# markdl/mtcp

Hardware: AMD Instinct MI355X
Metric: device-resident Gpkt/s + payload GB/s checksummed, 1/2/4/8 MI355X (higher is better)
Workload: dtype u8

## Files before the change

### mtcp_amd/csrc/dispatch.hpp

```cpp
#pragma once

#include <stdint.h>
#include <stdlib.h>
#include <string.h>

#include "../../include/mtcp_gpu.h"

namespace {

enum Sched : int { kSchedAuto = 0, kSchedWave, kSchedRow, kSchedQuad, kSchedBig, kSchedSpan, kSchedOct };

constexpr uint64_t kQuadOnlyUpToSlot = 64;
constexpr uint64_t kSpanUpToSlot = 640;
constexpr uint32_t kOctUpToPkts = 1u << 16;
constexpr uint64_t kOctUpToSlot = 2048;

inline int sched_from_env() {
    const char *e = getenv("MTCP_GPU_SCHED");
    if (!e) return kSchedAuto;
    if (!strcmp(e, "wave")) return kSchedWave;
    if (!strcmp(e, "row")) return kSchedRow;
    if (!strcmp(e, "quad")) return kSchedQuad;
    if (!strcmp(e, "span")) return kSchedSpan;
    if (!strcmp(e, "oct")) return kSchedOct;
    if (!strcmp(e, "big")) return kSchedBig;
    return kSchedAuto;
}

constexpr uint64_t kSpanNarrowUpToSlot = 896;
constexpr uint64_t kWaveNarrowUpToSlot = 4096;
constexpr uint32_t kWaveNarrowFromPkts = 1u << 20;

inline bool narrow_batch(const mtcp_gpu_size_hint *h) {
    if (!h || h->min_len == 0 || h->max_len < h->min_len) return false;
    const uint32_t lo = ((uint32_t)h->min_len + 63) & ~63u, hi = ((uint32_t)h->max_len + 63) & ~63u;
    return hi <= 2 * lo;
}

inline int pick_sched(int forced, uint32_t n, uint64_t slot, bool small_only, bool rx, bool narrow = false) {
    int s = forced;
    if (s == kSchedAuto) {
        int big = slot <= kQuadOnlyUpToSlot ? kSchedQuad
                  : slot <= kSpanUpToSlot   ? kSchedSpan
                  : (n <= kOctUpToPkts && slot <= kOctUpToSlot) ? kSchedOct : kSchedBig;
        if (narrow && slot > kQuadOnlyUpToSlot && slot <= kSpanUpToSlot && n <= kOctUpToPkts)
            big = kSchedOct;
        else if (narrow && slot > kSpanUpToSlot && slot <= kSpanNarrowUpToSlot && n > kOctUpToPkts)
            big = kSchedSpan;
        if (slot < 256) {
            s = n <= 2048 ? kSchedWave : n <= (1u << 17) ? kSchedQuad : big;
        } else if (narrow && slot <= kSpanUpToSlot && n > 2048 && n <= kOctUpToPkts) {
            s = kSchedOct;
        } else if (narrow && slot <= 320 && n > 2048 && n <= (1u << 17)) {
            s = kSchedQuad;
        } else if (slot >= 4096) {
            s = n <= (1u << 16) || (narrow && slot <= kWaveNarrowUpToSlot && n >= kWaveNarrowFromPkts)
                    ? kSchedWave : kSchedBig;
        } else {
            s = n <= 8192 || (slot >= 2048 && n <= 16384) ? kSchedWave
                : n <= (1u << 15)                          ? kSchedRow : big;
        }
    }
    if (s == kSchedSpan && !rx) s = kSchedBig;
    if (s == kSchedBig && small_only) s = kSchedRow;
    return s;
}

constexpr uint64_t kWaveShortUpToSlot = 2048;

constexpr uint64_t kUnrollBelowSlotBytes = 1024;
constexpr uint64_t kLineAlignAboveSlotBytes = 1536;
constexpr uint32_t kSortedUpToPkts = 1u << 16;

enum BigSched : int { kBigSorted = 0, kBigUnrolled, kBigUnrolledLineAligned, kBigSortedLineAligned };

inline int big_schedule(bool ptrs, uint64_t slot, uint32_t batch_n) {
    if (ptrs) return kBigSortedLineAligned;
    if (slot < kUnrollBelowSlotBytes || (batch_n <= kSortedUpToPkts && slot <= kLineAlignAboveSlotBytes))
        return kBigSorted;
    return slot > kLineAlignAboveSlotBytes ? kBigUnrolledLineAligned : kBigUnrolled;
}

inline const char *kernel_name(int sched, int big, uint64_t slot) {
    switch (sched) {
        case kSchedWave: return slot <= kWaveShortUpToSlot ? "rx_wave_kernel<2 loads>" : "rx_wave_kernel<10 loads>";
        case kSchedQuad: return "rx_group_kernel<quad>";
        case kSchedOct: return "rx_group_kernel<oct>";
        case kSchedSpan: return "rx_span_kernel";
        case kSchedRow: return "rx_group_kernel<row>";
        default: break;
    }
    switch (big) {
        case kBigSorted: return "rx_kernel<sorted>";
        case kBigUnrolled: return "rx_kernel<unrolled>";
        case kBigUnrolledLineAligned: return "rx_kernel<unrolled,line-aligned>";
        default: return "rx_kernel<sorted,line-aligned>";
    }
}

constexpr uint64_t kTxBuildOctUpToPayload = 48;
constexpr uint64_t kTxBuildRowUpToPayload = 384;
constexpr uint64_t kTxBuildHalfUpToPayload = 4096;
inline int txbuild_group(uint64_t payload_bytes, uint32_t n) {
    const uint64_t avg = n ? payload_bytes / n : 0;
    return avg <= kTxBuildOctUpToPayload    ? 8
           : avg <= kTxBuildRowUpToPayload  ? 16
           : avg <= kTxBuildHalfUpToPayload ? 32 : 64;
}

}
```

### mtcp_amd/csrc/mtcp_gpu.hip

```cpp
#include <hip/hip_runtime.h>
#include <stddef.h>
#include <stdint.h>
#include <string.h>

#include <algorithm>
#include <mutex>
#include <new>
#include <vector>

#include "../../include/mtcp_gpu.h"
#include "../../include/mtcp_gpu_flowtab.h"
#include "../../include/mtcp_gpu_group.h"
#include "../../include/mtcp_gpu_rcvwalk.h"
#include "../../include/mtcp_gpu_steer.h"
#include "../../include/mtcp_gpu_tcpopt.h"
#include "../../include/mtcp_gpu_txbuild.h"
#include "../../include/mtcp_gpu_txseg.h"
#include "ctx_internal.hpp"
#include "dispatch.hpp"
#include "flow_kernels.hpp"
#include "flowtab_kernels.hpp"
#include "group_kernels.hpp"
#include "host_call.hpp"
#include "host_copy.hpp"
#include "park.hpp"
#include "rcvwalk_kernels.hpp"
#include "rx_kernels.hpp"
#include "rx_span.hpp"
#include "steer_kernels.hpp"
#include "tcpopt_kernels.hpp"
#include "txbuild_kernels.hpp"
#include "txseg_kernels.hpp"
#include "wait.hpp"

namespace {

using namespace mtcp_host;
using mtcp_wait::Deadline;
using mtcp_wait::drain;

}

struct mtcp_gpu_ctx {
    int device = 0;
    int num_cu = 256;
    uint32_t flags = 0;
    uint32_t rss_nq = 1;
    uint32_t rss_endian = 0;
    uint32_t rss_key_w[4] = {0, 0, 0, 0};
    int sched = 0;
    hipStream_t stream = nullptr;
    const uint32_t *d_rss_tables = nullptr;
    uint32_t wait_us = 0;
    Stage stage[kStages];
    uint8_t *h_gather = nullptr;
    uint64_t h_gather_cap = 0;
    mtcp_gpu_desc *h_gather_desc = nullptr;
    uint32_t h_gather_desc_cap = 0;
    const char *last_kernel = "";
    bool abandoned = false;
};

namespace {

void build_rss_tables(const uint8_t key[40], uint32_t *tables) {
    uint32_t cache[96];
    uint32_t result = ((uint32_t)key[0] << 24) | ((uint32_t)key[1] << 16) |
                      ((uint32_t)key[2] << 8) | (uint32_t)key[3];
    uint32_t idx = 32;
    for (int i = 0; i < 96; i++, idx++) {
        cache[i] = result;
        const uint32_t bit = ((key[idx / 8] << (idx % 8)) & 0x80) ? 1u : 0u;
        result = (result << 1) | bit;
    }
    for (int t = 0; t < 24; ++t)
        for (int v = 0; v < 16; ++v) {
            uint32_t h = 0;
            for (int m = 0; m < 4; ++m)
                if (v & (0x8 >> m)) h ^= cache[4 * t + m];
            tables[t * 16 + v] = h;
        }
}

uint32_t grid_for(const mtcp_gpu_ctx *ctx, uint32_t n) {
    const uint32_t groups = (n + mg::kWave - 1) / mg::kWave;
    const uint32_t blocks = (groups + mg::kWavesPerBlock - 1) / mg::kWavesPerBlock;
    const uint32_t cap = (uint32_t)ctx->num_cu * 2;
    return std::max(1u, std::min(blocks, cap));
}

template <int SCHED, bool LALIGN>
constexpr int prio_for() { return SCHED == mg::kSchedUnrolled && !LALIGN ? 5 : 0; }

template <int MODE, bool RSS, int SCHED, bool LALIGN, bool CMP>
void launch_one(dim3 grid, dim3 block, hipStream_t st, const mg::KParams &kp) {
    constexpr bool kNT = MODE != mg::kTxChunk;
    constexpr bool kRev = LALIGN && SCHED == mg::kSchedUnrolled;
    constexpr int kB = SCHED == mg::kSchedSorted && !LALIGN && MODE == mg::kRxChunk ? 16 : 8;
    hipLaunchKernelGGL((mg::rx_kernel<MODE, RSS, SCHED, LALIGN, 0, 8, kB, kNT, 6, kRev, false,
                                      prio_for<SCHED, LALIGN>(), mg::kWavesPerBlock, 0, CMP>),
                       grid, block, 0, st, kp);
}

template <int MODE, bool RSS, bool CMP>
const char *launch_sched(dim3 grid, dim3 block, hipStream_t st, const mg::KParams &kp, uint64_t slot,
                         uint32_t batch_n) {
    const int b = big_schedule(MODE == mg::kRxPtrs, slot, batch_n);
    if constexpr (MODE == mg::kRxPtrs) {
        launch_one<MODE, RSS, mg::kSchedSorted, true, CMP>(grid, block, st, kp);
    } else if (b == kBigSorted) {
        launch_one<MODE, RSS, mg::kSchedSorted, false, CMP>(grid, block, st, kp);
    } else if (b == kBigUnrolledLineAligned) {
        launch_one<MODE, RSS, mg::kSchedUnrolled, true, CMP>(grid, block, st, kp);
    } else {
        launch_one<MODE, RSS, mg::kSchedUnrolled, false, CMP>(grid, block, st, kp);
    }
    return kernel_name(kSchedBig, b, slot);
}

constexpr uint32_t kHeldPasses = 8;


template <int MODE, bool RSS>
const char *launch_small(int sched, uint32_t n, uint64_t slot, hipStream_t st, const mg::KParams &kp) {
    if (sched == kSchedWave) {
        const dim3 grid((n + mg::kWavesPerBlock - 1) / mg::kWavesPerBlock);
        if (slot <= kWaveShortUpToSlot) {
            hipLaunchKernelGGL((mg::rx_wave_kernel<MODE, RSS, 0, 1, 2>), grid, dim3(mg::kBlock), 0, st, kp);
            return "rx_wave_kernel<2 loads>";
        }
        hipLaunchKernelGGL((mg::rx_wave_kernel<MODE, RSS>), grid, dim3(mg::kBlock), 0, st, kp);
        return "rx_wave_kernel<10 loads>";
    } else if (sched == kSchedQuad) {
        constexpr int kBlk = mg::kQuadBlock;
        constexpr uint32_t P = mg::GroupShape<4, kBlk>::P;
        hipLaunchKernelGGL((mg::rx_group_kernel<MODE, RSS, 4, 0, 1, kBlk>), dim3((n + P - 1) / P), dim3(kBlk), 0,
                           st, kp);
        return "rx_group_kernel<quad>";
    } else if (sched == kSchedOct) {
        constexpr int kBlk = mg::kOctBlock;
        constexpr uint32_t P = mg::GroupShape<8, kBlk>::P;
        hipLaunchKernelGGL((mg::rx_group_kernel<MODE, RSS, 8, 0, 1, kBlk>), dim3((n + P - 1) / P), dim3(kBlk), 0,
                           st, kp);
        return "rx_group_kernel<oct>";
    } else if (sched == kSchedSpan) {
        if constexpr (!mg::is_tx(MODE)) {
            hipLaunchKernelGGL((mg::rx_span_kernel<MODE, RSS>), dim3((n + mg::kSpanP - 1) / mg::kSpanP),
                               dim3(mg::kSpanBlock), 0, st, kp);
            return "rx_span_kernel";
        }
    }
    constexpr uint32_t P = mg::GroupShape<16>::P;
    hipLaunchKernelGGL((mg::rx_group_kernel<MODE, RSS, 16>), dim3((n + P - 1) / P), dim3(mg::kGroupBlock), 0,
                       st, kp);
    return "rx_group_kernel<row>";
}

uint64_t record_size(const mg::KParams &kp) { return kp.compact ? 16 : 40; }
uint64_t record_size(const mtcp_gpu_ctx *ctx) { return (ctx->flags & MTCP_GPU_F_COMPACT) ? 16 : 40; }

template <int MODE>
int launch(mtcp_gpu_ctx *ctx, const mg::KParams &kp, hipStream_t st, const mtcp_gpu_size_hint *hint = nullptr) {
    if (ctx->abandoned) return MTCP_GPU_EIO;
    if (kp.n == 0) return MTCP_GPU_OK;
    const bool rss = !mg::is_tx(MODE) && (ctx->flags & MTCP_GPU_F_RSS);
    const bool ptrs = MODE == mg::kRxPtrs || MODE == mg::kTxPtrs;
    const uint64_t avg_slot = ptrs ? 1024 : kp.buf_len / kp.n;
    const int sched = pick_sched(ctx->sched, kp.n, avg_slot, MODE == mg::kTxPtrs || kp.tx_report != nullptr,
                                 !mg::is_tx(MODE), !ptrs && narrow_batch(hint));
    if (sched != kSchedBig) {
        ctx->last_kernel = rss ? launch_small<MODE, true>(sched, kp.n, avg_slot, st, kp)
                               : launch_small<MODE, false>(sched, kp.n, avg_slot, st, kp);
        return HIP_OK(hipGetLastError()) ? MTCP_GPU_OK : MTCP_GPU_EIO;
    }
    if constexpr (MODE != mg::kTxPtrs) {
    const dim3 grid(grid_for(ctx, kp.n)), block(mg::kBlock);
    const uint64_t slot = kp.n ? kp.buf_len / kp.n : 0;
    const uint32_t cap = grid.x * mg::kWavesPerBlock * mg::kWave * kHeldPasses;
    for (uint32_t first = 0; first < kp.n; first += cap) {
        mg::KParams sub = kp;
        sub.n = std::min(kp.n - first, cap);
        if (MODE == mg::kRxPtrs) {
            sub.ptrs = kp.ptrs + first;
            sub.lens = kp.lens + first;
        } else {
            sub.desc = kp.desc + first;
        }
        if (MODE != mg::kTxChunk)
            sub.out = reinterpret_cast<mtcp_gpu_result *>(reinterpret_cast<uint8_t *>(kp.out) +
                                                          (uint64_t)first * record_size(kp));
        if (kp.bins) sub.bins = kp.bins + first;
        if constexpr (mg::is_tx(MODE)) {
            ctx->last_kernel = launch_sched<MODE, false, false>(grid, block, st, sub, slot, kp.n);
        } else if (kp.compact) {
            ctx->last_kernel = rss ? launch_sched<MODE, true, true>(grid, block, st, sub, slot, kp.n)
                                   : launch_sched<MODE, false, true>(grid, block, st, sub, slot, kp.n);
        } else {
            ctx->last_kernel = rss ? launch_sched<MODE, true, false>(grid, block, st, sub, slot, kp.n)
                                   : launch_sched<MODE, false, false>(grid, block, st, sub, slot, kp.n);
        }
    }
    }
    return HIP_OK(hipGetLastError()) ? MTCP_GPU_OK : MTCP_GPU_EIO;
}

mg::KParams base_params(mtcp_gpu_ctx *ctx) {
    mg::KParams kp{};
    kp.rss_tables = ctx->d_rss_tables;
    kp.rss_nq = ctx->rss_nq;
    kp.rss_endian = ctx->rss_endian;
    for (int i = 0; i < 4; ++i) kp.rss_key[i] = ctx->rss_key_w[i];
    kp.compact = (ctx->flags & MTCP_GPU_F_COMPACT) ? 1u : 0u;
    return kp;
}

uintptr_t out_align(const mtcp_gpu_ctx *ctx) { return (ctx->flags & MTCP_GPU_F_COMPACT) ? 15 : 7; }

hipStream_t pick(mtcp_gpu_ctx *ctx, void *stream) {
    return stream ? reinterpret_cast<hipStream_t>(stream) : ctx->stream;
}

void stage_release_buf(Stage &s, bool may_free) {
    mtcp_park::release(s.d_buf, s.buf_cap, mtcp_park::kDevice, may_free);
    s.d_buf = nullptr;
    s.buf_cap = 0;
}
void stage_release_pkts(Stage &s, bool may_free) {
    mtcp_park::release(s.d_desc, (size_t)s.pkt_cap * sizeof(mtcp_gpu_desc), mtcp_park::kDevice, may_free);
    mtcp_park::release(s.d_out, (size_t)s.pkt_cap * sizeof(mtcp_gpu_result), mtcp_park::kDevice, may_free);
    s.d_desc = nullptr;
    s.d_out = nullptr;
    s.pkt_cap = 0;
}
constexpr size_t kStageOptBytes = (size_t)kStagePkts * sizeof(mtcp_gpu_tcpopt);
void stage_release_opts(Stage &s, bool may_free) {
    mtcp_park::release(s.d_opt, kStageOptBytes, mtcp_park::kDevice, may_free);
    mtcp_park::release(s.h_opt, kStageOptBytes, mtcp_park::kHost, may_free);
    s.d_opt = s.h_opt = nullptr;
}
void stage_release_host(Stage &s, bool may_free) {
    mtcp_park::release(s.h_in, s.h_in_cap, mtcp_park::kHost, may_free);
    mtcp_park::release(s.h_out, s.h_out_cap, mtcp_park::kHost, may_free);
    s.h_in = s.h_out = nullptr;
    s.h_in_cap = s.h_out_cap = 0;
}

int waited(mtcp_gpu_ctx *ctx, int rc) {
    if (rc == MTCP_GPU_ETIMEDOUT) ctx->abandoned = true;
    return rc;
}

int stage_stream(mtcp_gpu_ctx *ctx, Stage &s) {
    if (s.stream) return MTCP_GPU_OK;
    if (&s == &ctx->stage[0]) {
        s.stream = ctx->stream;
        return MTCP_GPU_OK;
    }
    if (!HIP_OK(hipStreamCreateWithFlags(&s.stream, hipStreamNonBlocking))) return MTCP_GPU_EIO;
    s.own_stream = true;
    return MTCP_GPU_OK;
}

int stage_reserve(mtcp_gpu_ctx *ctx, Stage &s, uint64_t bytes, uint32_t pkts, const Deadline &dl) {
    if (ctx->abandoned) return MTCP_GPU_EIO;
    int rc = stage_stream(ctx, s);
    if (rc != MTCP_GPU_OK) return rc;
    if ((bytes > s.buf_cap || pkts > s.pkt_cap) && (rc = waited(ctx, drain(s.stream, dl))) != MTCP_GPU_OK)
        return rc;
    if (bytes > s.buf_cap) {
        stage_release_buf(s, !dl.bounded);
        const uint64_t cap = (bytes + 4095) & ~4095ull;
        if (!HIP_OK(mtcp_park::alloc(&s.d_buf, cap, mtcp_park::kDevice))) return MTCP_GPU_ENOMEM;
        s.buf_cap = cap;
    }
    if (pkts > s.pkt_cap) {
        stage_release_pkts(s, !dl.bounded);
        if (!HIP_OK(mtcp_park::alloc(&s.d_desc, (size_t)pkts * sizeof(mtcp_gpu_desc), mtcp_park::kDevice)))
            return MTCP_GPU_ENOMEM;
        if (!HIP_OK(mtcp_park::alloc(&s.d_out, (size_t)pkts * sizeof(mtcp_gpu_result), mtcp_park::kDevice))) {
            mtcp_park::release(s.d_desc, (size_t)pkts * sizeof(mtcp_gpu_desc), mtcp_park::kDevice, !dl.bounded);
            s.d_desc = nullptr;
            return MTCP_GPU_ENOMEM;
        }
// ... 1703 lines not shown
```

### mtcp_amd/csrc/rx_kernels.hpp

```cpp
#pragma once

#include <hip/hip_runtime.h>
#include <stdint.h>

#include <type_traits>

#include "../../include/mtcp_gpu.h"

namespace mg {

constexpr int kWave = 64;
constexpr int kBlock = 256;
constexpr int kWavesPerBlock = kBlock / kWave;
constexpr int kRssTableWords = 24 * 16;
constexpr int kSlotChunks = 8;
constexpr int kRow = 16;
constexpr int kUnroll = 6;

enum Mode : int { kRxChunk = 0, kRxPtrs = 1, kTxChunk = 2, kTxPtrs = 3 };
constexpr bool is_tx(int m) { return m == kTxChunk || m == kTxPtrs; }
enum Sched : int {
    kSchedRolled = 0,
    kSchedUnrolled = 3,
    kSchedSortedBase = 4,
    kSchedSortedEarly = 5,
    kSchedSorted = 6,
};

struct KParams {
    const uint8_t *buf;
    uint64_t buf_len;
    int64_t base_sub;
    const mtcp_gpu_desc *desc;
    const uint8_t *const *ptrs;
    const uint16_t *lens;
    uint32_t n;
    uint32_t off_shift;
    mtcp_gpu_result *out;
    const uint32_t *rss_tables;
    uint32_t rss_nq;
    uint32_t rss_endian;
    uint32_t *fill_count;
    uint32_t *bins;
    uint2 *tx_report;
    uint32_t *stamps;
    uint32_t rss_key[4];
    uint32_t compact;
};

typedef unsigned int v4u __attribute__((ext_vector_type(4)));

typedef __attribute__((address_space(1))) const v4u gv4u;
__device__ __forceinline__ v4u gload(uint64_t addr) { return *reinterpret_cast<gv4u *>(addr); }
__device__ __forceinline__ v4u gload_nt(uint64_t addr) {
    return __builtin_nontemporal_load(reinterpret_cast<gv4u *>(addr));
}
__device__ __forceinline__ uint4 gload4(uint64_t addr) {
    const v4u v = gload(addr);
    return make_uint4(v.x, v.y, v.z, v.w);
}

__device__ __forceinline__ uint32_t bswap16(uint32_t v) {
    return ((v & 0xFFu) << 8) | ((v >> 8) & 0xFFu);
}
__device__ __forceinline__ uint32_t bswap32(uint32_t v) { return __builtin_bswap32(v); }

__device__ __forceinline__ uint32_t halves(uint32_t d, uint32_t acc) {
    return __builtin_amdgcn_sad_u16(d, 0u, acc);
}
__device__ __forceinline__ uint32_t halves4(const v4u &v, uint32_t acc) {
    return halves(v.w, halves(v.z, halves(v.y, halves(v.x, acc))));
}

__device__ __forceinline__ uint32_t fold_csum(uint32_t s) {
    s = (s >> 16) + (s & 0xFFFFu);
    s += s >> 16;
    return (~s) & 0xFFFFu;
}

__device__ __forceinline__ uint32_t row_sum(uint32_t v) {
    v += (uint32_t)__builtin_amdgcn_update_dpp(0, (int)v, 0x111, 0xF, 0xF, true);
    v += (uint32_t)__builtin_amdgcn_update_dpp(0, (int)v, 0x112, 0xF, 0xF, true);
    v += (uint32_t)__builtin_amdgcn_update_dpp(0, (int)v, 0x114, 0xF, 0xF, true);
    v += (uint32_t)__builtin_amdgcn_update_dpp(0, (int)v, 0x118, 0xF, 0xF, true);
    return v;
}

__device__ __forceinline__ uint32_t shfl32(uint32_t v, int src) {
    return (uint32_t)__builtin_amdgcn_ds_bpermute(src << 2, (int)v);
}

__device__ __forceinline__ uint32_t row_bcast(uint32_t v, int i) {
#define MG_NB(n) case n: return (uint32_t)__builtin_amdgcn_update_dpp(0, (int)v, 0x150 + n, 0xF, 0xF, false)
    switch (i) {
        MG_NB(0); MG_NB(1); MG_NB(2); MG_NB(3); MG_NB(4); MG_NB(5); MG_NB(6); MG_NB(7);
        MG_NB(8); MG_NB(9); MG_NB(10); MG_NB(11); MG_NB(12); MG_NB(13); MG_NB(14);
        default: return (uint32_t)__builtin_amdgcn_update_dpp(0, (int)v, 0x15F, 0xF, 0xF, false);
    }
#undef MG_NB
}

__host__ __device__ __forceinline__ uint32_t hash_flow32(const uint32_t (&w)[3]) {
    uint32_t h = 0;
#pragma unroll
    for (int i = 0; i < 12; ++i) {
        h += (uint32_t)(int32_t)(int8_t)(uint8_t)(w[i >> 2] >> (8 * (i & 3)));
        h += h << 10;
        h ^= h >> 6;
    }
    h += h << 3;
    h ^= h >> 11;
    h += h << 15;
    return h;
}

__device__ __forceinline__ uint32_t hash_flow(const uint32_t (&w)[3]) {
    return hash_flow32(w) & (MTCP_GPU_NUM_BINS_FLOWS - 1);
}

__device__ __forceinline__ void flow_key(uint32_t saddr, uint32_t daddr, uint32_t ports, uint32_t (&w)[3]) {
    w[0] = daddr;
    w[1] = saddr;
    w[2] = (ports >> 16) | (ports << 16);
}

__device__ __forceinline__ uint32_t flow_bin(uint32_t saddr, uint32_t daddr, uint32_t ports,
                                             uint32_t verdict) {
    uint32_t w[3];
    flow_key(saddr, daddr, ports, w);
    return verdict == MTCP_GPU_V_TCP_OK ? hash_flow(w) : MTCP_GPU_FLOW_NONE;
// ... 310 lines not shown
        finish_seg<MODE>(k, sum - s_out);
    }
    return k;
}

__device__ __forceinline__ void pack_record(const Pkt &k, uint32_t rss_hash, uint32_t rss_queue,
                                            uint32_t (&r)[10]) {
    r[0] = k.saddr;
    r[1] = k.daddr;
    r[2] = k.ports;
    r[3] = k.seq;
    r[4] = k.ack;
    r[5] = k.window | (k.ip_len << 16);
    r[6] = k.ip_csum | (k.tcp_csum << 16);
    r[7] = rss_hash;
    r[8] = k.payload_len | (k.ihl_doff << 16) | (k.flags << 24);
    r[9] = k.verdict | (rss_queue << 8) | (k.eth_type << 16);
}

__device__ __forceinline__ void pack_compact(const Pkt &k, uint32_t rss_hash, uint32_t rss_queue,
                                             uint32_t (&r)[4]) {
    r[0] = rss_hash;
    r[1] = k.ip_csum | (k.tcp_csum << 16);
    r[2] = k.payload_len | (k.ip_len << 16);
    r[3] = k.ihl_doff | (k.flags << 8) | (k.verdict << 16) | (rss_queue << 24);
}

__device__ __forceinline__ void store_record(const KParams &kp, uint32_t rec, const Pkt &k,
                                             uint32_t rss_hash, uint32_t rss_queue) {
    if (kp.compact) {
        uint32_t c[4];
        pack_compact(k, rss_hash, rss_queue, c);
        reinterpret_cast<uint4 *>(kp.out)[rec] = make_uint4(c[0], c[1], c[2], c[3]);
    } else {
        uint32_t r[10];
        pack_record(k, rss_hash, rss_queue, r);
        uint2 *o = reinterpret_cast<uint2 *>(kp.out + rec);
#pragma unroll
        for (int i = 0; i < 5; ++i) o[i] = make_uint2(r[2 * i], r[2 * i + 1]);
    }
}

__device__ __forceinline__ uint32_t toeplitz_tables(const uint32_t *tab, uint32_t saddr,
                                                    uint32_t daddr, uint32_t ports) {
    uint32_t hh = 0;
#pragma unroll
    for (int b = 0; b < 4; ++b) {
        const uint32_t sb = (saddr >> (8 * b)) & 0xFFu;
        const uint32_t db = (daddr >> (8 * b)) & 0xFFu;
        const uint32_t pb = (ports >> (8 * b)) & 0xFFu;
        hh ^= tab[((2 * b) << 4) | (sb >> 4)] ^ tab[((2 * b + 1) << 4) | (sb & 15)];
        hh ^= tab[((8 + 2 * b) << 4) | (db >> 4)] ^ tab[((9 + 2 * b) << 4) | (db & 15)];
        hh ^= tab[((16 + 2 * b) << 4) | (pb >> 4)] ^ tab[((17 + 2 * b) << 4) | (pb & 15)];
    }
    return hh;
}

__device__ __forceinline__ uint32_t rss_core(uint32_t hh, uint32_t nq, uint32_t endian) {
    uint32_t m = hh & 0x7Fu;
    if (endian) m ^= 3u;
    return m % nq;
}

struct Frame {
    uint64_t p;
    uint32_t L;
    bool ok, live;
    uint64_t p16;
    uint32_t nch;
    uint32_t r_nch, r_lo, r_hi;
};

struct Trip {
    int i;
    uint32_t c0, nj;
    uint64_t base;
    uint32_t col;
    uint32_t skip = 0;
    uint32_t k = 0, ntrip = 0;
};

template <int MODE, bool RSS, int SCHED, bool LALIGN = false, int ABL = 0, int DEFER = 8, int B = 8,
          bool NT = true, int U = 6, bool REV = false, bool STAMP = false, int PRIO = 0,
          int WPB = kWavesPerBlock, int XSKIP = 0, bool CMP = false, int WPE = 2, bool COOP = true>
__global__ __launch_bounds__(kWave * WPB) __attribute__((amdgpu_waves_per_eu(WPE))) void rx_kernel(KParams kp) {
#ifndef MTCP_GPU_TESTING
    static_assert(ABL == 0 && !STAMP && XSKIP == 0,
                  "rx_kernel's ABL / STAMP / XSKIP variants need a -DMTCP_GPU_TESTING build (tools/)");
#endif
    uint64_t t_start = 0;
    if constexpr (STAMP) t_start = __builtin_amdgcn_s_memrealtime();
    if constexpr ((PRIO & 3) > 0) {
        if (blockIdx.x >= gridDim.x / 2) __builtin_amdgcn_s_setprio(PRIO & 3);
    }
    __shared__ uint32_t rss_lds[RSS ? kRssTableWords : 1];
    __shared__ WaveLds lds[WPB];
    if constexpr (RSS) {
        for (int i = threadIdx.x; i < kRssTableWords; i += kWave * WPB) rss_lds[i] = kp.rss_tables[i];
        __syncthreads();
    }

    const uint32_t lane = threadIdx.x & (kWave - 1);
    const uint32_t row = lane >> 4, rlane = lane & (kRow - 1);
    const uint32_t wib = threadIdx.x >> 6;
    const uint32_t wave = blockIdx.x * WPB + wib;
    const uint32_t nwaves = gridDim.x * WPB;
    WaveLds &wl = lds[wib];
    const uint32_t pass_pkts = nwaves * kWave;
    auto map = [&](uint32_t l) -> uint32_t {
        return B == kWave ? wave * kWave + l : (l / B) * (nwaves * B) + wave * B + (l % B);
    };
    const uint32_t lane_off = map(lane);
    bool xskip_wave = false;
    if constexpr (XSKIP != 0) {
        const uint32_t xcc = (uint32_t)__builtin_amdgcn_s_getreg((3 << 11) | 20) & 1u;
        xskip_wave = XSKIP > 0 ? xcc == 1u : xcc == 0u;
    }
    const uint64_t safe = (uint64_t)(uintptr_t)(MODE == kRxPtrs ? (const void *)kp.out
                                                               : (const void *)kp.buf);
    auto lane_pkt = [&](uint32_t g0, bool &live) -> uint32_t {
        live = g0 + lane_off < kp.n;
        return g0 + lane_off;
    };

    constexpr bool kCoop = B == 8 && MODE != kRxPtrs && SCHED == 3 && COOP;
    __shared__ uint64_t coop_a[kCoop ? 2 : 1][kCoop ? WPB * kWave : 1];
    uint32_t coop_buf = 0;

    const uint32_t cq = wib * kWave + lane, cj = cq / (8 * WPB), cidx = cq % (8 * WPB);
    const uint32_t coop_off = cj * (nwaves * 8) + blockIdx.x * (8 * WPB) + cidx;
    const uint32_t coop_slot = (cidx / 8) * kWave + cj * 8 + (cidx % 8);
    uint64_t raw_a = 0;
    uint32_t raw_b = 0;
    uint64_t cv_a = 0;
    auto fetch = [&](uint32_t g0) {
        if constexpr (kCoop) {
            const uint32_t kk = g0 + coop_off;
            if (kk < kp.n) cv_a = *reinterpret_cast<const uint64_t *>(kp.desc + kk);
            return;
        }
        bool live;
        const uint32_t k = lane_pkt(g0, live);
        if (live) {
            if constexpr (MODE == kRxPtrs) {
                raw_a = (uint64_t)(uintptr_t)kp.ptrs[k];
                raw_b = kp.lens[k];
            } else {
                raw_a = *reinterpret_cast<const uint64_t *>(kp.desc + k);
            }
        }
    };
    auto exchange = [&]() {
        if constexpr (kCoop) {
            coop_a[coop_buf][coop_slot] = cv_a;
            __syncthreads();
            raw_a = coop_a[coop_buf][wib * kWave + lane];
            coop_buf ^= 1u;
        }
    };
    auto decode = [&](uint32_t g0) -> Frame {
        Frame f;
        bool live;
        (void)lane_pkt(g0, live);
        f.live = live;
        if constexpr (XSKIP != 0) {
            if (xskip_wave && g0 + pass_pkts >= kp.n && lane >= (uint32_t)(kWave - (XSKIP > 0 ? XSKIP : -XSKIP)))
                f.live = false;
        }
        f.p = safe;
        f.L = 0;
        f.ok = false;
        if (f.live) {
            if constexpr (MODE == kRxPtrs) {
                f.L = raw_b;
                f.ok = raw_a != 0 && (raw_a & 1) == 0;
                if (f.ok) f.p = raw_a;
            } else {
                const uint32_t off = (uint32_t)raw_a;
                f.L = (uint32_t)(raw_a >> 32) & 0xFFFFu;
                const int64_t pos = (int64_t)((uint64_t)off << kp.off_shift) - kp.base_sub;
                f.ok = pos >= 0 && (pos & 1) == 0 && (uint64_t)pos + f.L <= kp.buf_len;
                if (f.ok) f.p = safe + (uint64_t)pos;
            }
        }
        f.p16 = f.p & ~15ull;
        f.nch = f.ok && f.L ? (uint32_t)((((f.p + f.L + 15) & ~15ull) - f.p16) >> 4) : 0u;
        const int src = 4 * (int)rlane + (int)row;
        f.r_nch = shfl32(f.nch, src);
        f.r_lo = shfl32((uint32_t)f.p16, src);
        f.r_hi = shfl32((uint32_t)(f.p16 >> 32), src);
        return f;
    };

    auto line_align = [&](Trip &t) {
        t.skip = 0;
        if constexpr (LALIGN) {
            if (t.nj > (uint32_t)(U * kRow)) {
                t.skip = (uint32_t)((t.base & 127) >> 4);
                t.base -= 16ull * t.skip;
                t.nj += t.skip;
            }
        }
    };
    auto enter_round = [&](const Frame &f, Trip &t, int ii) {
        t.i = ii;
        t.col = 4 * (uint32_t)ii + row;
        t.nj = row_bcast(f.r_nch, ii);
        t.base = ((uint64_t)row_bcast(f.r_hi, ii) << 32) | row_bcast(f.r_lo, ii);
        t.c0 = 0;
        line_align(t);
        if constexpr (REV) {
            t.k = 0;
            t.ntrip = (t.nj + U * kRow - 1) / (U * kRow);
            if ((row & 1) && t.ntrip > 1) t.c0 = (t.ntrip - 1) * (U * kRow);
        }
    };
    auto rev_step = [&](Trip &t) {
        ++t.k;
        t.c0 = t.k >= t.ntrip ? t.nj
               : (row & 1) ? (t.ntrip - 1 - t.k) * (U * kRow) : t.k * (U * kRow);
    };
    auto advance = [&](const Frame &f, Trip &t) -> bool {
        if (__ballot(t.c0 + U * kRow < t.nj)) {
            t.c0 += U * kRow;
            return true;
        }
        for (int ii = t.i + 1; ii < kWave / 4; ++ii) {
            enter_round(f, t, ii);
            if (__ballot(t.nj != 0)) return true;
        }
        t.nj = 0;
        return false;
    };
    auto first_trip = [&](const Frame &f, Trip &t) -> bool {
        enter_round(f, t, 0);
        return __ballot(t.nj != 0) || advance(f, t);
    };
    auto issue = [&](const Trip &t, v4u (&x)[U]) {
#pragma unroll
        for (int u = 0; u < U; ++u) {
            const uint32_t c = t.c0 + u * kRow + rlane;
            const uint32_t cc = c < t.nj ? c : (t.nj ? t.nj - 1 : 0u);
            x[u] = NT ? gload_nt(t.base + 16ull * cc) : gload(t.base + 16ull * cc);
        }
    };
    auto consume = [&](const Trip &t, const v4u (&x)[U], uint32_t &acc) {
        const uint32_t j = t.col;
        const uint32_t c_hd = rlane - t.skip;
        if (ABL < 2 && t.c0 == 0 && c_hd < kSlotChunks - 1) {
// ... 23 lines not shown
        nL = (uint32_t)__popcll(mb);
        nS = (uint32_t)__popcll(ms);
        const uint64_t below = (1ull << lane) - 1;
        const uint4 e = make_uint4((uint32_t)fr.p16, (uint32_t)(fr.p16 >> 32), fr.nch, lane);
        if (big) wl.info[__popcll(mb & below)] = e;
        if (sml) wl.info[kWave - 1 - __popcll(ms & below)] = e;
    };
    auto big_trip = [&](uint32_t nL, uint32_t ii, Trip &t) {
        const uint32_t r = 4 * ii + row;
        t.i = (int)ii;
        t.c0 = 0;
        t.skip = 0;
        t.nj = 0;
        t.base = safe;
        t.col = kWave;
        if (r < nL) {
            const uint4 e = wl.info[r];
            t.base = ((uint64_t)e.y << 32) | e.x;
            t.nj = e.z;
            t.col = e.w;
            line_align(t);
        }
    };
    auto small_trip = [&](uint32_t nS, uint32_t ii, Trip &t) {
        const uint32_t r = kQuads * ii + (lane >> 2);
        t.i = (int)ii;
        t.c0 = 0;
        t.skip = 0;
        t.nj = 0;
        t.base = safe;
        t.col = kWave;
        if (r < nS) {
            const uint4 e = wl.info[kWave - 1 - r];
            t.base = ((uint64_t)e.y << 32) | e.x;
            t.nj = e.z;
            t.col = e.w;
        }
    };
    auto small_load = [&](const Trip &t) -> v4u {
        const uint32_t q = lane & 3;
        const uint32_t cc = q < t.nj ? q : (t.nj ? t.nj - 1 : 0u);
        return NT && SCHED < 5 ? gload_nt(t.base + 16ull * cc) : gload(t.base + 16ull * cc);
    };
    auto small_finish = [&](const Trip &t, const v4u &v) {
        const uint32_t q = lane & 3;
        uint32_t s4 = q < t.nj ? halves4(v, 0u) : 0u;
        s4 += (uint32_t)__builtin_amdgcn_update_dpp(0, (int)s4, 0xB1, 0xF, 0xF, false);
        s4 += (uint32_t)__builtin_amdgcn_update_dpp(0, (int)s4, 0x4E, 0xF, 0xF, false);
        if (q == 0) wl.sum[t.col] = s4;
        if (q < t.nj) {
            uint32_t *d = wl.hd + 4 * q * kHdStride + t.col;
            d[0] = v.x; d[kHdStride] = v.y; d[2 * kHdStride] = v.z; d[3 * kHdStride] = v.w;
        }
        if (q + 1 == t.nj) {
            uint32_t *d = wl.hd + 4 * (kSlotChunks - 1) * kHdStride + t.col;
            d[0] = v.x; d[kHdStride] = v.y; d[2 * kHdStride] = v.z; d[3 * kHdStride] = v.w;
        }
    };

    constexpr int kDefer = MODE == kTxChunk ? 0 : DEFER;
    constexpr int RW = CMP ? 4 : 10, HW = CMP ? 5 : 10;
    uint32_t keep[kDefer > 0 ? kDefer : 1][HW];
    uint32_t held = 0;
    uint32_t last_g0 = 0;
    uint8_t *const out_b = reinterpret_cast<uint8_t *>(kp.out);
    auto flush = [&]() {
        if constexpr (kDefer > 0) {
            static_assert(B % 2 == 0, "16 B pieces need runs of an even number of records");
            constexpr uint32_t kRunDw = B * RW, kRunPieces = kRunDw / 4;
            uint32_t *stg = reinterpret_cast<uint32_t *>(&wl.hd[0]);
#pragma unroll
            for (int q = 0; q < kDefer; ++q) {
                if ((uint32_t)q < held) {
                    const uint32_t gq = last_g0 - (uint32_t)q * pass_pkts;
                    uint2 *st = reinterpret_cast<uint2 *>(stg) + lane * (RW / 2);
#pragma unroll
                    for (int i = 0; i < RW / 2; ++i) st[i] = make_uint2(keep[q][2 * i], keep[q][2 * i + 1]);
#pragma unroll
                    for (uint32_t pc = lane; pc < kWave * RW / 4; pc += kWave) {
                        const uint32_t run = pc / kRunPieces, w = pc % kRunPieces;
                        const uint32_t first = gq + map(run * B);
                        const uint32_t r0 = first + (4 * w) / RW, r1 = first + (4 * w + 2) / RW;
                        const uint4 v = *reinterpret_cast<const uint4 *>(stg + run * kRunDw + 4 * w);
                        uint8_t *dst = out_b + (uint64_t)first * (4 * RW) + 16 * w;
                        if (r1 < kp.n) {
                            *reinterpret_cast<uint4 *>(dst) = v;
                        } else if (r0 < kp.n) {
                            *reinterpret_cast<uint2 *>(dst) = make_uint2(v.x, v.y);
                        }
                    }
                    if (kp.bins) {
                        bool live;
                        const uint32_t rec = lane_pkt(gq, live);
                        if (live)
                            kp.bins[rec] = CMP ? keep[q][HW - 1]
                                               : flow_bin(keep[q][0], keep[q][1], keep[q][2], keep[q][9] & 0xFFu);
                    }
                }
            }
            held = 0;
        }
    };

    auto push = [&](const uint32_t (&r)[HW], uint32_t g0) {
        if constexpr (kDefer > 0) {
            if (held == (uint32_t)kDefer) flush();
#pragma unroll
            for (int q = kDefer - 1; q > 0; --q)
#pragma unroll
                for (int i = 0; i < HW; ++i) keep[q][i] = keep[q - 1][i];
#pragma unroll
            for (int i = 0; i < HW; ++i) keep[0][i] = r[i];
            last_g0 = g0;
            ++held;
        }
    };

    constexpr int kTxDefer = MODE == kTxChunk && DEFER > 0 ? DEFER : 0;
    uint32_t tkeep[kTxDefer > 0 ? kTxDefer : 1][4];
    uint32_t tx_held = 0;
    auto tx_write = [&](const uint32_t (&w)[4]) {
        if (w[3]) {
            uint16_t *q16 = reinterpret_cast<uint16_t *>(((uint64_t)w[1] << 32) | w[0]);
            q16[12] = (uint16_t)w[2];
            q16[(w[3] + 16) >> 1] = (uint16_t)(w[2] >> 16);
        }
    };
    auto tx_flush = [&]() {
        if constexpr (kTxDefer > 0) {
#pragma unroll
            for (int q = 0; q < kTxDefer; ++q)
                if ((uint32_t)q < tx_held) tx_write(tkeep[q]);
            tx_held = 0;
        }
    };
    auto tx_push = [&](const uint32_t (&w)[4]) {
        if constexpr (kTxDefer > 0) {
            if (tx_held == (uint32_t)kTxDefer) tx_flush();
#pragma unroll
            for (int q = kTxDefer - 1; q > 0; --q)
#pragma unroll
                for (int i = 0; i < 4; ++i) tkeep[q][i] = tkeep[q - 1][i];
#pragma unroll
            for (int i = 0; i < 4; ++i) tkeep[0][i] = w[i];
            ++tx_held;
        }
    };

    fetch(0);
    exchange();
    v4u X[U], Y[U];
    Trip pre;
    bool have_pre = false;
    Trip sa, sb;
    v4u va, vb;
    bool have_pre_small = false;
    for (uint32_t g0 = 0; g0 < kp.n; g0 += pass_pkts) {
        if constexpr ((PRIO & 4) != 0) {
            if (g0 == 4 * pass_pkts) __builtin_amdgcn_s_setprio(0);
        }
        const Frame f = decode(g0);
        if (!__ballot(f.live)) break;
        fetch(g0 + pass_pkts);
        const uint32_t k = g0 + lane_off;
        const bool live = f.live, desc_ok = f.ok;
        const uint64_t p = f.p;
        const uint32_t L = f.L, nch = f.nch;
        const bool has_next = g0 + pass_pkts < kp.n;

        if constexpr (SCHED >= 4) {
            uint32_t nL, nS;
            if (!have_pre) prepare(f, nL, nS);
            else nL = pre_nL, nS = pre_nS;
            const uint32_t RL = (nL + 3) / 4, RS = (nS + kQuads - 1) / kQuads;
            uint32_t acc = 0;
            auto finish_big = [&](Trip &t, const v4u (&cb)[U]) {
                consume(t, cb, acc);
                while (__ballot(t.c0 + U * kRow < t.nj)) {
                    t.c0 += U * kRow;
                    v4u Z[U];
                    issue(t, Z);
                    consume(t, Z, acc);
                }
                acc = row_sum(acc);
                if (rlane == kRow - 1) wl.sum[t.col] = acc;
                acc = 0;
            };
            if constexpr (SCHED >= 5) {
                if (have_pre_small) {
                } else if (RL > 0 && !have_pre) {
                    Trip t0;
                    big_trip(nL, 0, t0);
                    issue(t0, X);
                    pre = t0;
                    have_pre = true;
                }
                if (!have_pre_small) {
                    small_trip(nS, 0, sa);
                    small_trip(nS, 1, sb);
                    va = small_load(sa);
                    vb = small_load(sb);
                }
                have_pre_small = false;
            }
            if (RL > 0) {
                Trip cur, nxt;
                if (have_pre) {
                    cur = pre;
                } else {
                    big_trip(nL, 0, cur);
                    issue(cur, X);
                }
                for (uint32_t i = 0; i < RL; i += 2) {
                    if (i + 1 < RL) {
                        big_trip(nL, i + 1, nxt);
                        issue(nxt, Y);
                    }
                    finish_big(cur, X);
                    if (i + 1 >= RL) break;
                    if (i + 2 < RL) {
                        big_trip(nL, i + 2, cur);
                        issue(cur, X);
                    }
                    finish_big(nxt, Y);
                }
            }
            have_pre = false;
            uint32_t s0 = 0;
            if constexpr (SCHED >= 5) {
                if (RS > 0) {
                    small_finish(sa, va);
                    small_finish(sb, vb);
                }
                s0 = 2;
            }
            for (uint32_t i = s0; i < RS; i += 2) {
                Trip a, b;
                small_trip(nS, i, a);
                small_trip(nS, i + 1, b);
                const v4u va = small_load(a), vb = small_load(b);
                small_finish(a, va);
                small_finish(b, vb);
            }
            if (has_next) {
                exchange();
                const Frame fn = decode(g0 + pass_pkts);
                prepare(fn, pre_nL, pre_nS);
                if constexpr (SCHED == 6) {
                    small_trip(pre_nS, 0, sa);
                    small_trip(pre_nS, 1, sb);
                    va = small_load(sa);
// ... 3 lines not shown
                if (pre_nL) {
                    big_trip(pre_nL, 0, pre);
                    issue(pre, X);
                    have_pre = true;
                }
            }
        } else if constexpr (SCHED == 3) {
            uint32_t acc = 0;
            static_for<0, kWave / 4>([&](auto I) {
                constexpr int i = decltype(I)::value;
                Trip t;
                enter_round(f, t, i);
                if (i > 0 || !have_pre) issue(t, X);
                consume(t, X, acc);
                if constexpr (REV) {
                    while (__ballot(t.k + 1 < t.ntrip)) {
                        rev_step(t);
                        issue(t, X);
                        consume(t, X, acc);
                    }
                } else {
                    while (__ballot(t.c0 + U * kRow < t.nj)) {
                        t.c0 += U * kRow;
                        issue(t, X);
                        consume(t, X, acc);
                    }
                }
                acc = row_sum(acc);
                if (rlane == kRow - 1) wl.sum[4 * i + (int)row] = acc;
                acc = 0;
            });
            have_pre = false;
            if (has_next) {
                exchange();
                const Frame fn = decode(g0 + pass_pkts);
                Trip n;
                enter_round(fn, n, 0);
                issue(n, X);
                have_pre = true;
            }
        } else {
            Trip cur;
            bool have;
            if (have_pre) {
                cur = pre;
                have = true;
            } else {
                have = first_trip(f, cur);
                issue(cur, X);
            }
            have_pre = false;
            uint32_t acc = 0;
            while (have) {
                Trip n = cur;
                const bool more = advance(f, n);
                consume(cur, X, acc);
                if (!more || n.i != cur.i) {
                    acc = row_sum(acc);
                    if (rlane == kRow - 1) wl.sum[4 * cur.i + (int)row] = acc;
                    acc = 0;
                }
                if (!more) break;
                issue(n, X);
                cur = n;
            }
            if (has_next) {
                Trip n;
                exchange();
                const Frame fn = decode(g0 + pass_pkts);
                if (__ballot(fn.live) && first_trip(fn, n)) {
                    issue(n, X);
                    pre = n;
                    have_pre = true;
                }
            }
        }

        if constexpr (ABL >= 1) {
            if constexpr (kDefer > 0) {
                uint32_t r[HW] = {};
                r[0] = wl.sum[lane];
                push(r, g0);
            } else if (live && wl.sum[lane] == 0x12345678u) {
                kp.out[k].saddr = wl.sum[lane];
            }
            continue;
        }
        const Pkt pk = parse_finish<MODE, kHdStride>(wl.hd + lane, wl.sum[lane], p, L, nch, desc_ok);
        uint32_t rss_hash = 0, rss_queue = 0;
        if constexpr (RSS) {
            if (pk.tcp_entry) {
                rss_hash = toeplitz_tables(rss_lds, pk.saddr, pk.daddr, pk.ports);
                rss_queue = rss_core(rss_hash, kp.rss_nq, kp.rss_endian);
            }
        }

        if constexpr (MODE == kTxChunk) {
            uint32_t fill[4] = {0, 0, 0, 0};
            if (live && pk.need_sum) {
                const uint32_t ipc = fold_csum(pk.s_ip - pk.ip_check);
                fill[0] = (uint32_t)p;
                fill[1] = (uint32_t)(p >> 32);
                fill[2] = ipc | (pk.tcp_csum << 16);
                fill[3] = pk.T;
                if (kp.fill_count) atomicAdd(kp.fill_count, 1u);
            }
            if constexpr (kTxDefer > 0) {
                tx_push(fill);
            } else {
                tx_write(fill);
            }
        } else {
            uint32_t r[HW];
            if constexpr (CMP) {
                uint32_t c[4];
                pack_compact(pk, rss_hash, rss_queue, c);
#pragma unroll
                for (int i = 0; i < 4; ++i) r[i] = c[i];
                r[4] = kp.bins ? flow_bin(pk.saddr, pk.daddr, pk.ports, pk.verdict) : 0u;
            } else {
                pack_record(pk, rss_hash, rss_queue, r);
            }
            if constexpr (kDefer > 0) {
                push(r, g0);
            } else {
                uint2 *st = reinterpret_cast<uint2 *>(wl.hd) + lane * (RW / 2);
#pragma unroll
                for (int i = 0; i < RW / 2; ++i) st[i] = make_uint2(r[2 * i], r[2 * i + 1]);
                const uint2 *src = reinterpret_cast<const uint2 *>(wl.hd);
#pragma unroll
                for (uint32_t i = 0; i < RW / 2; ++i) {
                    const uint32_t q = i * kWave + lane;
                    const uint32_t rec = g0 + map(q / (RW / 2));
                    if (rec < kp.n)
                        reinterpret_cast<uint2 *>(out_b + (uint64_t)rec * (4 * RW))[q % (RW / 2)] = src[q];
                }
                if (kp.bins && live)
                    kp.bins[k] = CMP ? r[HW - 1] : flow_bin(r[0], r[1], r[2], r[9] & 0xFFu);
            }
        }
    }
    flush();
    tx_flush();
    if constexpr (STAMP) {
        __builtin_amdgcn_s_waitcnt(0);
        const uint64_t t_end = __builtin_amdgcn_s_memrealtime();
        if (lane == 0) {
            uint32_t *st = kp.stamps + 4 * wave;
            st[0] = (uint32_t)t_start;
            st[1] = (uint32_t)t_end;
            st[2] = (uint32_t)__builtin_amdgcn_s_getreg((3 << 11) | 20);
            st[3] = (uint32_t)__builtin_amdgcn_s_getreg((31 << 11) | 4);
        }
    }
}

}
```

Baseline: 6625.

## Launch all partitions of a large batch in one kernel grid

Large batches used to be split into several sequential kernel launches, each covering grid*waves*64*held packets. Now a single launch covers every partition: the grid becomes part_blocks*parts and each block works out its partition offset, packet count and block index from blockIdx, with pointers offset by pfirst. The goal is to cut per-launch overhead and the serialization gaps between partition launches, and to let partitions overlap on the device. Non-final partitions write records through buffer-resource stores with a bounds-checked range. The kRxPtrs path still uses multiple launches.

```diff
diff --git a/mtcp_amd/csrc/dispatch.hpp b/mtcp_amd/csrc/dispatch.hpp
--- a/mtcp_amd/csrc/dispatch.hpp
+++ b/mtcp_amd/csrc/dispatch.hpp
@@ -81,6 +81,50 @@
     return slot > kLineAlignAboveSlotBytes ? kBigUnrolledLineAligned : kBigUnrolled;
 }
 
+struct PartGeom {
+    uint32_t part_pkts;
+    uint32_t part_blocks;
+    uint32_t parts;
+};
+
+inline PartGeom part_geom(uint32_t n, uint32_t blocks, uint32_t wpb, uint32_t held) {
+    PartGeom g;
+    g.part_blocks = blocks;
+    g.part_pkts = blocks * wpb * 64u * held;
+    g.parts = n ? (uint32_t)(((uint64_t)n + g.part_pkts - 1) / g.part_pkts) : 1u;
+    return g;
+}
+
+struct PartOwner {
+    uint32_t block;
+    uint32_t wib;
+    uint32_t lane;
+    uint32_t pass;
+};
+
+inline PartOwner part_owner(const PartGeom &g, uint32_t wpb, uint32_t B, uint32_t k) {
+    const uint32_t part = k / g.part_pkts, local = k - part * g.part_pkts;
+    const uint32_t W = g.part_blocks * wpb, pass_pkts = W * 64u;
+    const uint32_t r = local % pass_pkts;
+    const uint32_t wave = (r % (W * B)) / B;
+    PartOwner o;
+    o.block = part * g.part_blocks + wave / wpb;
+    o.wib = wave % wpb;
+    o.lane = (r / (W * B)) * B + r % B;
+    o.pass = local / pass_pkts;
+    return o;
+}
+
+inline uint32_t part_packet(const PartGeom &g, uint32_t wpb, uint32_t B, uint32_t n, const PartOwner &o) {
+    const uint32_t part = o.block / g.part_blocks, bid = o.block - part * g.part_blocks;
+    const uint64_t first = (uint64_t)part * g.part_pkts;
+    if (first >= n) return UINT32_MAX;
+    const uint32_t part_n = n - (uint32_t)first < g.part_pkts ? n - (uint32_t)first : g.part_pkts;
+    const uint32_t W = g.part_blocks * wpb, wave = bid * wpb + o.wib;
+    const uint64_t local = (uint64_t)o.pass * (W * 64u) + (o.lane / B) * (W * B) + wave * B + o.lane % B;
+    return local < part_n ? (uint32_t)(first + local) : UINT32_MAX;
+}
+
 inline const char *kernel_name(int sched, int big, uint64_t slot) {
     switch (sched) {
         case kSchedWave: return slot <= kWaveShortUpToSlot ? "rx_wave_kernel<2 loads>" : "rx_wave_kernel<10 loads>";
diff --git a/mtcp_amd/csrc/mtcp_gpu.hip b/mtcp_amd/csrc/mtcp_gpu.hip
--- a/mtcp_amd/csrc/mtcp_gpu.hip
+++ b/mtcp_amd/csrc/mtcp_gpu.hip
@@ -92,33 +92,34 @@
 template <int SCHED, bool LALIGN>
 constexpr int prio_for() { return SCHED == mg::kSchedUnrolled && !LALIGN ? 5 : 0; }
 
-template <int MODE, bool RSS, int SCHED, bool LALIGN, bool CMP>
+template <int MODE, bool RSS, int SCHED, bool LALIGN, bool CMP, int PARTS>
 void launch_one(dim3 grid, dim3 block, hipStream_t st, const mg::KParams &kp) {
     constexpr bool kNT = MODE != mg::kTxChunk;
     constexpr bool kRev = LALIGN && SCHED == mg::kSchedUnrolled;
     constexpr int kB = SCHED == mg::kSchedSorted && !LALIGN && MODE == mg::kRxChunk ? 16 : 8;
     hipLaunchKernelGGL((mg::rx_kernel<MODE, RSS, SCHED, LALIGN, 0, 8, kB, kNT, 6, kRev, false,
-                                      prio_for<SCHED, LALIGN>(), mg::kWavesPerBlock, 0, CMP>),
+                                      prio_for<SCHED, LALIGN>(), mg::kWavesPerBlock, 0, CMP, 2, true, PARTS>),
                        grid, block, 0, st, kp);
 }
 
-template <int MODE, bool RSS, bool CMP>
+template <int MODE, bool RSS, bool CMP, int PARTS>
 const char *launch_sched(dim3 grid, dim3 block, hipStream_t st, const mg::KParams &kp, uint64_t slot,
                          uint32_t batch_n) {
     const int b = big_schedule(MODE == mg::kRxPtrs, slot, batch_n);
     if constexpr (MODE == mg::kRxPtrs) {
-        launch_one<MODE, RSS, mg::kSchedSorted, true, CMP>(grid, block, st, kp);
+        launch_one<MODE, RSS, mg::kSchedSorted, true, CMP, PARTS>(grid, block, st, kp);
     } else if (b == kBigSorted) {
-        launch_one<MODE, RSS, mg::kSchedSorted, false, CMP>(grid, block, st, kp);
+        launch_one<MODE, RSS, mg::kSchedSorted, false, CMP, PARTS>(grid, block, st, kp);
     } else if (b == kBigUnrolledLineAligned) {
-        launch_one<MODE, RSS, mg::kSchedUnrolled, true, CMP>(grid, block, st, kp);
+        launch_one<MODE, RSS, mg::kSchedUnrolled, true, CMP, PARTS>(grid, block, st, kp);
     } else {
-        launch_one<MODE, RSS, mg::kSchedUnrolled, false, CMP>(grid, block, st, kp);
+        launch_one<MODE, RSS, mg::kSchedUnrolled, false, CMP, PARTS>(grid, block, st, kp);
     }
     return kernel_name(kSchedBig, b, slot);
 }
 
 constexpr uint32_t kHeldPasses = 8;
+constexpr int kPartsMode = 3;
 
 
 template <int MODE, bool RSS>
@@ -159,6 +160,21 @@
 uint64_t record_size(const mg::KParams &kp) { return kp.compact ? 16 : 40; }
 uint64_t record_size(const mtcp_gpu_ctx *ctx) { return (ctx->flags & MTCP_GPU_F_COMPACT) ? 16 : 40; }
 
+template <int MODE, int PARTS>
+const char *launch_parts(bool rss, dim3 grid, dim3 block, hipStream_t st, const mg::KParams &kp, uint64_t slot,
+                         uint32_t batch_n = 0) {
+    if (!batch_n) batch_n = kp.n;
+    if constexpr (mg::is_tx(MODE)) {
+        return launch_sched<MODE, false, false, PARTS>(grid, block, st, kp, slot, batch_n);
+    } else if (kp.compact) {
+        return rss ? launch_sched<MODE, true, true, PARTS>(grid, block, st, kp, slot, batch_n)
+                   : launch_sched<MODE, false, true, PARTS>(grid, block, st, kp, slot, batch_n);
+    } else {
+        return rss ? launch_sched<MODE, true, false, PARTS>(grid, block, st, kp, slot, batch_n)
+                   : launch_sched<MODE, false, false, PARTS>(grid, block, st, kp, slot, batch_n);
+    }
+}
+
 template <int MODE>
 int launch(mtcp_gpu_ctx *ctx, const mg::KParams &kp, hipStream_t st, const mtcp_gpu_size_hint *hint = nullptr) {
     if (ctx->abandoned) return MTCP_GPU_EIO;
@@ -176,29 +192,25 @@
     if constexpr (MODE != mg::kTxPtrs) {
     const dim3 grid(grid_for(ctx, kp.n)), block(mg::kBlock);
     const uint64_t slot = kp.n ? kp.buf_len / kp.n : 0;
-    const uint32_t cap = grid.x * mg::kWavesPerBlock * mg::kWave * kHeldPasses;
-    for (uint32_t first = 0; first < kp.n; first += cap) {
-        mg::KParams sub = kp;
-        sub.n = std::min(kp.n - first, cap);
-        if (MODE == mg::kRxPtrs) {
+    const PartGeom pg = part_geom(kp.n, grid.x, mg::kWavesPerBlock, kHeldPasses);
+    if (pg.parts == 1) {
+        ctx->last_kernel = launch_parts<MODE, 0>(rss, grid, block, st, kp, slot);
+    } else if constexpr (MODE == mg::kRxPtrs) {
+        for (uint32_t first = 0; first < kp.n; first += pg.part_pkts) {
+            mg::KParams sub = kp;
+            sub.n = std::min(kp.n - first, pg.part_pkts);
             sub.ptrs = kp.ptrs + first;
             sub.lens = kp.lens + first;
-        } else {
-            sub.desc = kp.desc + first;
-        }
-        if (MODE != mg::kTxChunk)
             sub.out = reinterpret_cast<mtcp_gpu_result *>(reinterpret_cast<uint8_t *>(kp.out) +
                                                           (uint64_t)first * record_size(kp));
-        if (kp.bins) sub.bins = kp.bins + first;
-        if constexpr (mg::is_tx(MODE)) {
-            ctx->last_kernel = launch_sched<MODE, false, false>(grid, block, st, sub, slot, kp.n);
-        } else if (kp.compact) {
-            ctx->last_kernel = rss ? launch_sched<MODE, true, true>(grid, block, st, sub, slot, kp.n)
-                                   : launch_sched<MODE, false, true>(grid, block, st, sub, slot, kp.n);
-        } else {
-            ctx->last_kernel = rss ? launch_sched<MODE, true, false>(grid, block, st, sub, slot, kp.n)
-                                   : launch_sched<MODE, false, false>(grid, block, st, sub, slot, kp.n);
+            if (kp.bins) sub.bins = kp.bins + first;
+            ctx->last_kernel = launch_parts<MODE, 0>(rss, grid, block, st, sub, slot, kp.n);
         }
+    } else {
+        mg::KParams all = kp;
+        all.part_pkts = pg.part_pkts;
+        all.part_blocks = pg.part_blocks;
+        ctx->last_kernel = launch_parts<MODE, kPartsMode>(rss, dim3(pg.part_blocks * pg.parts), block, st, all, slot);
     }
     }
     return HIP_OK(hipGetLastError()) ? MTCP_GPU_OK : MTCP_GPU_EIO;
diff --git a/mtcp_amd/csrc/rx_kernels.hpp b/mtcp_amd/csrc/rx_kernels.hpp
--- a/mtcp_amd/csrc/rx_kernels.hpp
+++ b/mtcp_amd/csrc/rx_kernels.hpp
@@ -46,6 +46,8 @@
     uint32_t *stamps;
     uint32_t rss_key[4];
     uint32_t compact;
+    uint32_t part_pkts;
+    uint32_t part_blocks;
 };
 
 typedef unsigned int v4u __attribute__((ext_vector_type(4)));
@@ -522,7 +524,8 @@
 
 template <int MODE, bool RSS, int SCHED, bool LALIGN = false, int ABL = 0, int DEFER = 8, int B = 8,
           bool NT = true, int U = 6, bool REV = false, bool STAMP = false, int PRIO = 0,
-          int WPB = kWavesPerBlock, int XSKIP = 0, bool CMP = false, int WPE = 2, bool COOP = true>
+          int WPB = kWavesPerBlock, int XSKIP = 0, bool CMP = false, int WPE = 2, bool COOP = true,
+          int PARTS = 0>
 __global__ __launch_bounds__(kWave * WPB) __attribute__((amdgpu_waves_per_eu(WPE))) void rx_kernel(KParams kp) {
 #ifndef MTCP_GPU_TESTING
     static_assert(ABL == 0 && !STAMP && XSKIP == 0,
@@ -530,8 +533,16 @@
 #endif
     uint64_t t_start = 0;
     if constexpr (STAMP) t_start = __builtin_amdgcn_s_memrealtime();
+    uint32_t bid = blockIdx.x, nblk = gridDim.x, pfirst = 0, pn = kp.n;
+    if constexpr ((PARTS & 1) != 0) {
+        const uint32_t part = blockIdx.x / kp.part_blocks;
+        nblk = kp.part_blocks;
+        bid = blockIdx.x - part * nblk;
+        pfirst = part * kp.part_pkts;
+        pn = kp.n - pfirst < kp.part_pkts ? kp.n - pfirst : kp.part_pkts;
+    }
     if constexpr ((PRIO & 3) > 0) {
-        if (blockIdx.x >= gridDim.x / 2) __builtin_amdgcn_s_setprio(PRIO & 3);
+        if (bid >= nblk / 2 && ((PARTS & 4) == 0 || pfirst == 0)) __builtin_amdgcn_s_setprio(PRIO & 3);
     }
     __shared__ uint32_t rss_lds[RSS ? kRssTableWords : 1];
     __shared__ WaveLds lds[WPB];
@@ -543,8 +554,8 @@
     const uint32_t lane = threadIdx.x & (kWave - 1);
     const uint32_t row = lane >> 4, rlane = lane & (kRow - 1);
     const uint32_t wib = threadIdx.x >> 6;
-    const uint32_t wave = blockIdx.x * WPB + wib;
-    const uint32_t nwaves = gridDim.x * WPB;
+    const uint32_t wave = bid * WPB + wib;
+    const uint32_t nwaves = nblk * WPB;
     WaveLds &wl = lds[wib];
     const uint32_t pass_pkts = nwaves * kWave;
     auto map = [&](uint32_t l) -> uint32_t {
@@ -559,7 +570,7 @@
     const uint64_t safe = (uint64_t)(uintptr_t)(MODE == kRxPtrs ? (const void *)kp.out
                                                                : (const void *)kp.buf);
     auto lane_pkt = [&](uint32_t g0, bool &live) -> uint32_t {
-        live = g0 + lane_off < kp.n;
+        live = g0 + lane_off < pn;
         return g0 + lane_off;
     };
 
@@ -568,7 +579,7 @@
     uint32_t coop_buf = 0;
 
     const uint32_t cq = wib * kWave + lane, cj = cq / (8 * WPB), cidx = cq % (8 * WPB);
-    const uint32_t coop_off = cj * (nwaves * 8) + blockIdx.x * (8 * WPB) + cidx;
+    const uint32_t coop_off = cj * (nwaves * 8) + bid * (8 * WPB) + cidx;
     const uint32_t coop_slot = (cidx / 8) * kWave + cj * 8 + (cidx % 8);
     uint64_t raw_a = 0;
     uint32_t raw_b = 0;
@@ -576,17 +587,17 @@
     auto fetch = [&](uint32_t g0) {
         if constexpr (kCoop) {
             const uint32_t kk = g0 + coop_off;
-            if (kk < kp.n) cv_a = *reinterpret_cast<const uint64_t *>(kp.desc + kk);
+            if (kk < pn) cv_a = *reinterpret_cast<const uint64_t *>(kp.desc + pfirst + kk);
             return;
         }
         bool live;
         const uint32_t k = lane_pkt(g0, live);
         if (live) {
             if constexpr (MODE == kRxPtrs) {
-                raw_a = (uint64_t)(uintptr_t)kp.ptrs[k];
-                raw_b = kp.lens[k];
+                raw_a = (uint64_t)(uintptr_t)kp.ptrs[pfirst + k];
+                raw_b = kp.lens[pfirst + k];
             } else {
-                raw_a = *reinterpret_cast<const uint64_t *>(kp.desc + k);
+                raw_a = *reinterpret_cast<const uint64_t *>(kp.desc + pfirst + k);
             }
         }
     };
@@ -604,7 +615,7 @@
         (void)lane_pkt(g0, live);
         f.live = live;
         if constexpr (XSKIP != 0) {
-            if (xskip_wave && g0 + pass_pkts >= kp.n && lane >= (uint32_t)(kWave - (XSKIP > 0 ? XSKIP : -XSKIP)))
+            if (xskip_wave && g0 + pass_pkts >= pn && lane >= (uint32_t)(kWave - (XSKIP > 0 ? XSKIP : -XSKIP)))
                 f.live = false;
         }
         f.p = safe;
@@ -794,10 +805,15 @@
                         const uint32_t first = gq + map(run * B);
                         const uint32_t r0 = first + (4 * w) / RW, r1 = first + (4 * w + 2) / RW;
                         const uint4 v = *reinterpret_cast<const uint4 *>(stg + run * kRunDw + 4 * w);
-                        uint8_t *dst = out_b + (uint64_t)first * (4 * RW) + 16 * w;
-                        if (r1 < kp.n) {
+                        uint8_t *dst = out_b + (uint64_t)(pfirst + first) * (4 * RW) + 16 * w;
+                        if ((PARTS & 2) != 0 && kp.n - pfirst > pn) {
+                            const __amdgpu_buffer_rsrc_t rs = __builtin_amdgcn_make_buffer_rsrc(
+                                out_b + (uint64_t)pfirst * (4 * RW), 0, (int)(pn * (4 * RW)), 0x00027000);
+                            __builtin_amdgcn_raw_buffer_store_b128(v4u{v.x, v.y, v.z, v.w}, rs,
+                                                                   (int)(first * (4 * RW) + 16 * w), 0, 16);
+                        } else if (r1 < pn) {
                             *reinterpret_cast<uint4 *>(dst) = v;
-                        } else if (r0 < kp.n) {
+                        } else if (r0 < pn) {
                             *reinterpret_cast<uint2 *>(dst) = make_uint2(v.x, v.y);
                         }
                     }
@@ -805,7 +821,7 @@
                         bool live;
                         const uint32_t rec = lane_pkt(gq, live);
                         if (live)
-                            kp.bins[rec] = CMP ? keep[q][HW - 1]
+                            kp.bins[pfirst + rec] = CMP ? keep[q][HW - 1]
                                                : flow_bin(keep[q][0], keep[q][1], keep[q][2], keep[q][9] & 0xFFu);
                     }
                 }
@@ -867,7 +883,7 @@
     Trip sa, sb;
     v4u va, vb;
     bool have_pre_small = false;
-    for (uint32_t g0 = 0; g0 < kp.n; g0 += pass_pkts) {
+    for (uint32_t g0 = 0; g0 < pn; g0 += pass_pkts) {
         if constexpr ((PRIO & 4) != 0) {
             if (g0 == 4 * pass_pkts) __builtin_amdgcn_s_setprio(0);
         }
@@ -878,7 +894,7 @@
         const bool live = f.live, desc_ok = f.ok;
         const uint64_t p = f.p;
         const uint32_t L = f.L, nch = f.nch;
-        const bool has_next = g0 + pass_pkts < kp.n;
+        const bool has_next = g0 + pass_pkts < pn;
 
         if constexpr (SCHED >= 4) {
             uint32_t nL, nS;
@@ -1048,7 +1064,7 @@
                 r[0] = wl.sum[lane];
                 push(r, g0);
             } else if (live && wl.sum[lane] == 0x12345678u) {
-                kp.out[k].saddr = wl.sum[lane];
+                kp.out[pfirst + k].saddr = wl.sum[lane];
             }
             continue;
         }
@@ -1098,11 +1114,11 @@
                 for (uint32_t i = 0; i < RW / 2; ++i) {
                     const uint32_t q = i * kWave + lane;
                     const uint32_t rec = g0 + map(q / (RW / 2));
-                    if (rec < kp.n)
-                        reinterpret_cast<uint2 *>(out_b + (uint64_t)rec * (4 * RW))[q % (RW / 2)] = src[q];
+                    if (rec < pn)
+                        reinterpret_cast<uint2 *>(out_b + (uint64_t)(pfirst + rec) * (4 * RW))[q % (RW / 2)] = src[q];
                 }
                 if (kp.bins && live)
-                    kp.bins[k] = CMP ? r[HW - 1] : flow_bin(r[0], r[1], r[2], r[9] & 0xFFu);
+                    kp.bins[pfirst + k] = CMP ? r[HW - 1] : flow_bin(r[0], r[1], r[2], r[9] & 0xFFu);
             }
         }
     }
```

Result: slower. 6551 (-1.1%).
